# jyakaranda/A-LeGO-LOAM

Measured on AMD Instinct MI355X. Metric: scans/sec (16x1800 LiDAR) full IP->LO->LM loop, higher is better.
Workload: dtype f32/f64

## Files before the change

a-lego-loam_amd/csrc/alego_api.hip:

```cpp
#include <hip/hip_runtime.h>

#include <cmath>
#include <cstdio>
#include <cstdlib>
#include <algorithm>
#include <cstring>
#include <mutex>
#include <set>
#include <string>
#include <vector>

#include "../../include/alego_mi355x.h"
#include "dev_common.h"
#include "dev_mem.h"
#include "front_end.h"
#include "lm_ctx.h"
#include "lm_host.h"
#include "merge_math.h"
#include "thin_math.h"
#include "loop_ctx.h"
#include "pgraph.h"
#include "prof.h"
#include "reloc.h"
#include "stream_plan.h"
// ... 160 lines not shown
    h->gsize = h->plan.gsize;
    const int G = h->plan.groups;
    for (int g = 0; g < G; ++g) {
      hipStream_t s = nullptr;
      if (hipStreamCreate(&s) != hipSuccess) { for (hipStream_t t : h->streams) hipStreamDestroy(t); delete h; return ALEGO_ERR_HIP; }
      h->streams.push_back(s);
    }
    h->stream = h->streams[0];
    h->lm_async = h->plan.async != 0;
    if (h->lm_async) {
      for (int g = 0; g < G; ++g) {
        hipStream_t s = nullptr;
        hipEvent_t e[4] = {nullptr, nullptr, nullptr, nullptr};
        bool ok = hipStreamCreate(&s) == hipSuccess;
        for (int k = 0; k < 4 && ok; ++k) ok = hipEventCreateWithFlags(&e[k], hipEventDisableTiming) == hipSuccess;
        if (!ok) { h->lm_async = false; break; }
        h->back.push_back(s);
        h->ev_stage.push_back(e[0]); h->ev_stage.push_back(e[1]); h->ev_back.push_back(e[2]); h->ev_back.push_back(e[3]);
      }
      h->grp_scans.assign(G, 0);
    }
  }
  DevCtx& d = h->d;
  std::memset(&d, 0, sizeof(d));
  d.P = *params;
  d.n_slots = n_slots; d.ring_len = ring_len; d.slot0 = 0; d.n_launch = n_slots;
  d.fs_cur = d.fs_last = -1;
  d.NS = params->n_scan; d.H = params->horizon_scan; d.N = d.NS * d.H; d.Pcap = d.N;
  d.cap_sharp = params->n_sharp * params->n_sectors;
  d.cap_lsharp = params->n_less_sharp * params->n_sectors;
  d.cap_flat = params->n_flat * params->n_sectors;
  d.st_stride = d.cap_sharp + d.cap_lsharp + d.cap_flat + d.H;
  d.sin_ax = std::sin(params->seg_alpha_x); d.cos_ax = std::cos(params->seg_alpha_x);
  d.sin_ay = std::sin(params->seg_alpha_y); d.cos_ay = std::cos(params->seg_alpha_y);
  {
    const double lo = params->sensor_mount_ang - params->ground_angle_thres, hi = params->sensor_mount_ang + params->ground_angle_thres;
    const bool ok = lo > -89.0 && hi < 89.0 && lo < hi;
    d.tan_g_lo = ok ? std::tan(lo * M_PI / 180.0) : std::nan("");
    d.tan_g_hi = ok ? std::tan(hi * M_PI / 180.0) : std::nan("");
  }
  d.h_magic = (unsigned)((1ull << 32) / (unsigned long long)d.H) + 1u;
  d.inv_res_x = 1.0 / params->ang_res_x; d.inv_res_y = 1.0 / params->ang_res_y;
  d.tan_theta = (params->seg_theta > 0.0 && params->seg_theta < 1.5) ? std::tan(params->seg_theta) : std::nan("");
  d.opt_ip_screen = env_int("ALEGO_IP_SCREEN", 1) != 0;
  d.ip_scr = ip_screen_consts(d.sin_ax, d.cos_ax, d.sin_ay, d.cos_ay, d.tan_theta, d.tan_g_lo, d.tan_g_hi, d.opt_ip_screen);
  d.opt_ip_fused = env_int("ALEGO_IP_FUSED", 1) != 0;
  d.opt_ip_half = env_int("ALEGO_IP_HALF", 1) != 0;
  d.opt_cc_fused = env_int("ALEGO_CC_FUSED", 1) != 0;
  d.opt_cc_tile = env_int("ALEGO_CC_TILE", 1) != 0;
  d.opt_ip_band = env_int("ALEGO_IP_BAND", 1) != 0;
  d.opt_fe_pick1 = env_int("ALEGO_FE_PICK1", 0) != 0;
  d.opt_fe_fused = env_int("ALEGO_FE_FUSED", 1) != 0;
  d.opt_fe_cand = env_int("ALEGO_FE_CAND", 0);
  d.opt_lo_box_lds = env_int("ALEGO_LO_BOX_LDS", 1 << 20);
  d.opt_lo_grid = env_int("ALEGO_LO_GRID", 1) != 0;
  d.opt_fo_spin = env_int("ALEGO_FE_SPIN", 0);
  d.opt_fo_pad8 = env_int("ALEGO_FE_PAD8", 0) != 0;
  d.opt_map_merge = env_int("ALEGO_MAP_MERGE", 1) != 0;
  d.opt_solve_full_eval = env_int("ALEGO_SOLVE_FULL_EVAL", 0) != 0;
  d.fcap[F_SHARP] = d.cap_sharp * d.NS; d.fcap[F_LSHARP] = d.cap_lsharp * d.NS; d.fcap[F_FLAT] = d.cap_flat * d.NS; d.fcap[F_LFLAT] = d.N;
  d.lo_qcap_surf = d.fcap[F_FLAT]; d.lo_qcap_corner = d.fcap[F_SHARP];
  d.lo_box_cap = (d.N + LO_CH - 1) / LO_CH + d.NS;
  const size_t B = n_slots, N = d.N, NS = d.NS;
  int rc = 0;
  rc |= dalloc(h, &d.in_pts, B * ring_len * d.Pcap, false);
  rc |= dalloc(h, &d.in_n, B * ring_len);
  rc |= dalloc(h, &d.owner, B * N); rc |= dalloc(h, &d.range_img, B * N); rc |= dalloc(h, &d.flag_img, B * N);
  rc |= dalloc(h, &d.parent, B * N); rc |= dalloc(h, &d.cc_size, B * N); rc |= dalloc(h, &d.cc_rows, B * N);
  rc |= dalloc(h, &d.label_img, B * N); rc |= dalloc(h, &d.cc_label, B * N);
  d.ipb_col = nullptr; d.ipb_off = nullptr;
  if (d.NS > 16 && d.NS <= 64) { rc |= dalloc(h, &d.ipb_col, B * ipb_col_n(d)); rc |= dalloc(h, &d.ipb_off, B * ipb_off_n(d)); }
  d.ipf_own = nullptr;
  if (d.NS <= 16 && d.N <= 65535 && (d.H & 1) == 0) rc |= dalloc(h, &d.ipf_own, B * (N / 2), false);
  rc |= dalloc(h, &d.seg_pts, B * N); rc |= dalloc(h, &d.seg_ground, B * N); rc |= dalloc(h, &d.seg_col, B * N);
  rc |= dalloc(h, &d.seg_range, B * N); rc |= dalloc(h, &d.outlier, B * N);
  rc |= dalloc(h, &d.cd, B * N); rc |= dalloc(h, &d.picked0, B * N); rc |= dalloc(h, &d.fe_flag, B * N); rc |= dalloc(h, &d.plabel, B * N);
  rc |= fe_store_alloc(d, B, [&](auto** p, size_t n, bool zero) { return dalloc(h, p, n, zero); });
  rc |= dalloc(h, &d.scan_stamp, B);
  rc |= dalloc(h, &d.seg_dsk, h->P.deskew_mode ? B * N : 1);
  {
    const double rx = params->ang_res_x, ry = params->ang_res_y;
    std::vector<double> rt(2 * (NS + 6)), ct;
    for (int k = 0; k < (int)NS + 6; ++k) {
      const double phi = (((double)(k - 3) - 0.5) * ry - params->ang_bottom) * M_PI / 180.0;
      rt[2 * k] = std::cos(phi); rt[2 * k + 1] = std::sin(phi);
    }
    d.ip_cmin = (int)std::floor(180.0 / rx) - 2;
    d.ip_ncb = (int)std::floor(540.0 / rx) + 3 - d.ip_cmin;
    ct.resize(2 * (size_t)d.ip_ncb);
    for (int k = 0; k < d.ip_ncb; ++k) {
      const double A = (double)(d.ip_cmin + k) * rx * M_PI / 180.0;
      ct[2 * k] = std::cos(A); ct[2 * k + 1] = std::sin(A);
    }
    double2 *rtd = nullptr, *ctd = nullptr;
    rc |= dalloc(h, &rtd, NS + 6); rc |= dalloc(h, &ctd, (size_t)d.ip_ncb);
    if (!rc && (hipMemcpy(rtd, rt.data(), rt.size() * sizeof(double), hipMemcpyHostToDevice) != hipSuccess ||
                hipMemcpy(ctd, ct.data(), ct.size() * sizeof(double), hipMemcpyHostToDevice) != hipSuccess)) { h->err = "upload of the projection tables failed"; rc = ALEGO_ERR_HIP; }
    d.ip_rowtab = rtd; d.ip_coltab = ctd;
    {
      std::vector<double> cf(d.H);
      for (int c = 0; c < d.H; ++c) cf[c] = c / 10000.0;
      double* cfd = nullptr;
      rc |= dalloc(h, &cfd, (size_t)d.H);
      if (!rc && hipMemcpy(cfd, cf.data(), cf.size() * sizeof(double), hipMemcpyHostToDevice) != hipSuccess) { h->err = "upload of the column table failed"; rc = ALEGO_ERR_HIP; }
      d.ip_colfrac = cfd;
    }
// ... 641 lines not shown
  DevPool T;
  double *dg, *dp, *dr, *dj;
  HIP_TRY(h, T.get(&dg, (size_t)n * 13, false)); HIP_TRY(h, T.get(&dp, 6, false)); HIP_TRY(h, T.get(&dr, (size_t)n, false)); HIP_TRY(h, T.get(&dj, (size_t)n * 6, false));
  HIP_TRY(h, hipMemcpy(dg, geom13, (size_t)n * 13 * 8, hipMemcpyHostToDevice));
  HIP_TRY(h, hipMemcpy(dp, params6, 48, hipMemcpyHostToDevice));
  launch_dbg_eval_blocks(type, n, dg, dp, dr, dj, h->stream);
  HIP_TRY(h, hipStreamSynchronize(h->stream));
  HIP_TRY(h, hipMemcpy(res, dr, (size_t)n * 8, hipMemcpyDeviceToHost));
  HIP_TRY(h, hipMemcpy(jac6, dj, (size_t)n * 48, hipMemcpyDeviceToHost));
  return 0;
}

int alego_debug_transform_to_start(alego_handle* h, const double* params6, const alego_point* pts, int n, alego_point* out) {
  if (!h || n < 0 || !params6 || (n > 0 && (!pts || !out))) return ALEGO_ERR_ARG;
  if (n == 0) return 0;
  hipSetDevice(h->device);
  DevPool T;
  double* dp;
  float4 *di, *dout;
  HIP_TRY(h, T.get(&dp, 6, false)); HIP_TRY(h, T.get(&di, (size_t)n, false)); HIP_TRY(h, T.get(&dout, (size_t)n, false));
  HIP_TRY(h, hipMemcpy(dp, params6, 48, hipMemcpyHostToDevice));
  HIP_TRY(h, hipMemcpy(di, pts, (size_t)n * 16, hipMemcpyHostToDevice));
  launch_dbg_transform_to_start(dp, di, n, dout, h->stream);
  HIP_TRY(h, hipStreamSynchronize(h->stream));
  HIP_TRY(h, hipMemcpy(out, dout, (size_t)n * 16, hipMemcpyDeviceToHost));
  return 0;
}

int alego_debug_check_guards(char* report, int cap) {
  std::string r;
  const int bad = guard_check(&r);
  if (report && cap > 0) { std::strncpy(report, r.c_str(), (size_t)cap - 1); report[cap - 1] = 0; }
  return bad;
}

int alego_debug_set_option(alego_handle* h, const char* name, int value) {
  if (!h || !name) return ALEGO_ERR_ARG;
  const std::string s(name);
  DevCtx& d = h->d;
  if (s == "ALEGO_CC_FUSED") d.opt_cc_fused = value != 0;
  else if (s == "ALEGO_IP_FUSED") d.opt_ip_fused = value != 0;
  else if (s == "ALEGO_IP_HALF") d.opt_ip_half = value != 0;
  else if (s == "ALEGO_IP_SCREEN") { d.opt_ip_screen = value != 0; d.ip_scr = ip_screen_consts(d.sin_ax, d.cos_ax, d.sin_ay, d.cos_ay, d.tan_theta, d.tan_g_lo, d.tan_g_hi, d.opt_ip_screen); }
  else if (s == "ALEGO_CC_TILE") d.opt_cc_tile = value != 0;
  else if (s == "ALEGO_IP_BAND") {
    HIP_TRY(h, hipDeviceSynchronize());
    HIP_TRY(h, hipMemset(d.cc_size, 0, (size_t)d.n_slots * d.N * sizeof(int)));
    HIP_TRY(h, hipMemset(d.cc_rows, 0, (size_t)d.n_slots * d.N * sizeof(unsigned long long)));
    d.opt_ip_band = value != 0;
  }
  else if (s == "ALEGO_FE_PICK1") d.opt_fe_pick1 = value != 0;
  else if (s == "ALEGO_FE_FUSED") d.opt_fe_fused = value != 0;
  else if (s == "ALEGO_FE_CAND") d.opt_fe_cand = value;
  else if (s == "ALEGO_LO_BOX_LDS") d.opt_lo_box_lds = value;
  else if (s == "ALEGO_LO_GRID") d.opt_lo_grid = value != 0;
  else if (s == "ALEGO_FE_SPIN") d.opt_fo_spin = value;
  else if (s == "ALEGO_SOLVE_FULL_EVAL") d.opt_solve_full_eval = value != 0;
  else if (s == "ALEGO_FE_PAD8") d.opt_fo_pad8 = value != 0;
  else if (s == "ALEGO_FE_ERR_CLEAR") {
    if (value < -1 || value >= d.n_slots) return ALEGO_ERR_ARG;
    HIP_TRY(h, hipDeviceSynchronize());
    if (value >= 0) HIP_TRY(h, hipMemset(scal_of(d, value) + SC_FE_ERR, 0, 4));
    else HIP_TRY(h, hipMemset2D(scal_of(d, 0) + SC_FE_ERR, scal_n() * sizeof(int), 0, 4, d.n_slots));
  }
  else if (s == "ALEGO_MAP_MERGE") { if (int r = lm_host_set_map_merge(h->lm, value != 0, &h->err)) return r; d.opt_map_merge = value != 0; }
  else if (s == "ALEGO_IP_FAST") d.ip_fast = h->ip_fast_capable & value;
  else if (s == "ALEGO_POKE_GUARD") { HIP_TRY(h, hipMemset(scal_of(d, d.n_slots) + value, 0xFF, 4)); }
  else if (s == "ALEGO_GV_SMALL_MAX") { HIP_TRY(h, sync_all(h)); return lm_host_set_gv_small_max(h->lm, value); }
  else if (s == "ALEGO_PG_BUDGET") graph_ctx_set_budget(&h->pg, value);
  else if (s == "ALEGO_LC_BUDGET") loop_ctx_set_budget(&h->lc, value);
  else if (s == "ALEGO_RL_BUDGET") reloc_ctx_set(&h->rl, 0, value);
  else if (s == "ALEGO_RL_BRUTE") reloc_ctx_set(&h->rl, 1, value);
  else if (s == "ALEGO_SHARD_SLICE") return lm_host_debug_slice(h->lm, value & 0xff, value >> 8, &h->err);
  else { h->err = "unknown option " + s; return ALEGO_ERR_ARG; }
  return 0;
}

int alego_loop_detect(const alego_params* P, const float* keyposes6, const double* stamps, int32_t n, const double cur_xyz[3]) {
  if (!P || n <= 0 || !keyposes6 || !stamps || !cur_xyz) return -1;
  const float cx = (float)cur_xyz[0], cy = (float)cur_xyz[1], cz = (float)cur_xyz[2];
  const float r2 = (float)(P->lc_search_radius * P->lc_search_radius);
  std::vector<std::pair<float, int>> cand;
  for (int i = 0; i < n; ++i) {
    float r = 0.f, df;
    df = keyposes6[i * 6 + 0] - cx; r += df * df; df = keyposes6[i * 6 + 1] - cy; r += df * df; df = keyposes6[i * 6 + 2] - cz; r += df * df;
    if (r < r2) cand.emplace_back(r, i);
  }
  std::sort(cand.begin(), cand.end());
  for (const auto& c : cand)
    if (stamps[n - 1] - stamps[c.second] > P->lc_min_time_gap) return c.second;
  return -1;
}
int alego_loop_closure_icp(alego_handle* h, const alego_kf_in* latest, const alego_kf_in* history, int32_t n_history, alego_icp_result* out,
                           alego_point* target_out, int32_t target_cap) {
  if (!h || !latest || !out || n_history < 0 || (n_history > 0 && !history)) return ALEGO_ERR_ARG;
  hipSetDevice(h->device);
  g_prof = &h->prof;
  return icp_run(h->P, latest, history, n_history, out, target_out, target_out ? target_cap : 0, h->stream, &h->err);
}

int alego_loop_search(alego_handle* h, const int32_t* slots, int32_t n, alego_loop_result* out) {
  if (!h || n < 0 || (n > 0 && (!slots || !out))) return ALEGO_ERR_ARG;
  if (!h->map_on) { h->err = "alego_loop_search: the key-frame archive is off (alego_map_enable)"; return ALEGO_ERR_ARG; }
  for (int i = 0; i < n; ++i) if (slots[i] < 0 || slots[i] >= h->d.n_slots) { h->err = "alego_loop_search: slot out of range"; return ALEGO_ERR_ARG; }
  hipSetDevice(h->device);
  g_prof = &h->prof;
// ... 537 lines not shown
  hipSetDevice(h->device);
  return lm_host_map_stamps(h->lm, slot, first, n, const_cast<double*>(stamps), 1, &h->err);
}
int alego_map_keyposes(alego_handle* h, int slot, alego_point* out, int32_t cap) {
  if (int r = check_slot(h, slot)) return r;
  hipSetDevice(h->device);
  return lm_host_map_keyposes(h->lm, slot, out, cap, &h->err);
}
int alego_lm_get_local_map(alego_handle* h, int slot, alego_point* corner, int32_t corner_cap, alego_point* surf, int32_t surf_cap, int32_t n_out[2]) {
  if (int r = check_slot(h, slot)) return r;
  if (!n_out || corner_cap < 0 || surf_cap < 0) return ALEGO_ERR_ARG;
  hipSetDevice(h->device);
  return lm_host_get_local_map(h->lm, slot, corner, corner_cap, surf, surf_cap, n_out, &h->err);
}
int alego_voxel_grid(alego_handle* h, const alego_point* pts, int32_t n, float leaf, alego_point* out, int32_t cap) {
  if (!h || n < 0 || cap < 0 || (n > 0 && !pts) || !(leaf > 0.f)) return ALEGO_ERR_ARG;
  hipSetDevice(h->device);
  g_prof = &h->prof;
  return lm_host_voxel_grid(h->lm, h->stream, pts, n, leaf, out, cap, &h->err);
}

int alego_debug_get(alego_handle* h, int slot, const char* name, void* out, int cap_bytes, int* count, int* dtype) {
  if (int r = check_slot(h, slot)) return r;
  hipSetDevice(h->device);
  const DevCtx& d = h->d;
  int sc[SC_COUNT];
  HIP_TRY(h, hipMemcpyAsync(sc, scal_of(d, slot), sizeof(sc), hipMemcpyDeviceToHost, stream_of(h, slot)));
  HIP_TRY(h, hipStreamSynchronize(stream_of(h, slot)));
  const std::string s(name);
  if (s.rfind("la_", 0) == 0) {
    const void* rsrc = nullptr;
    size_t bytes = 0;
    if (loop_app_debug_get(h->rl, slot, name, &rsrc, &bytes)) { h->err = std::string("debug_get: ") + name + " needs alego_loop_appearance_enable"; return ALEGO_ERR_ARG; }
    if ((size_t)cap_bytes < bytes) { h->err = "debug_get: buffer too small"; return ALEGO_ERR_CAPACITY; }
    if (bytes) HIP_TRY(h, hipMemcpy(out, rsrc, bytes, hipMemcpyDeviceToHost));
    *count = (int)bytes; *dtype = 3;
    return 0;
  }
  if (s.rfind("rl_", 0) == 0) {
    if (s == "rl_stats") {
      if (cap_bytes < 8) { h->err = "debug_get: buffer too small"; return ALEGO_ERR_CAPACITY; }
      reloc_debug_stats(h->rl, (int*)out);
      *count = 2; *dtype = 2;
      return 0;
    }
    const void* rsrc = nullptr;
    size_t bytes = 0;
    if (reloc_debug_get(h->rl, slot, name, &rsrc, &bytes)) { h->err = std::string("debug_get: ") + name + " needs alego_reloc_enable"; return ALEGO_ERR_ARG; }
    if ((size_t)cap_bytes < bytes) { h->err = "debug_get: buffer too small"; return ALEGO_ERR_CAPACITY; }
    if (bytes) HIP_TRY(h, hipMemcpy(out, rsrc, bytes, hipMemcpyDeviceToHost));
    *count = (int)bytes; *dtype = 3;
    return 0;
  }
  const size_t base = (size_t)slot * d.N, M = sc[SC_M];
  const size_t fb = fbuf(slot, sc[SC_CUR]);
  int fc[F_KINDS];
  HIP_TRY(h, hipMemcpy(fc, feat_cnt_of(d, fb), sizeof(fc), hipMemcpyDeviceToHost));
  static const char* const cloud[F_KINDS] = {"sharp", "less_sharp", "flat", "less_flat"};
  struct Row { std::string name; const void* row; size_t n; int dtype; };
  std::vector<Row> tab = {
    {"range_img", d.range_img + base, (size_t)d.N, 0}, {"label_img", d.label_img + base, (size_t)d.N, 2}, {"flag_img", d.flag_img + base, (size_t)d.N, 3},
    {"owner", d.owner + base, (size_t)d.N, 2}, {"parent", d.parent + base, (size_t)d.N, 2},
    {"seg_cloud", d.seg_pts + base, M * 4, 0}, {"outlier", d.outlier + base, (size_t)sc[SC_NOUT] * 4, 0},
    {"imu_ptr", imu_ptr_of(d, slot), IMP_N, 2}, {"imu_ring", imu_ring_of(d, slot), imu_ring_n(), 1},
    {"seg_ground", d.seg_ground + base, M, 3}, {"seg_col", d.seg_col + base, M, 2}, {"seg_range", d.seg_range + base, M, 0},
    {"ring_start", ring_start_of(d, slot, 0), (size_t)d.NS, 2}, {"ring_end", ring_end_of(d, slot, 0), (size_t)d.NS, 2},
    {"orientation", ori_of(d, slot), ORI_N, 0}, {"scal", scal_of(d, slot), SC_COUNT, 2},
    {"curv_d", d.cd + base, M, 0}, {"picked_occl", d.picked0 + base, M, 3}, {"point_label", d.plabel + base, M, 2},
    {"lo_surf_corr", lo_corr_of(d, slot, 0), (size_t)fc[F_FLAT] * LC_W, 2}, {"lo_corner_corr", lo_corr_of(d, slot, 1), (size_t)fc[F_SHARP] * LC_W, 2},
    {"lo_state", lo_state_of(d, slot), LO_STATE_N, 1}, {"poses", poses_of(d, slot), PO_W, 1}};
  if (d.P.deskew_mode) tab.push_back({"undistorted", d.seg_dsk + base, (size_t)sc[SC_M_DSK] * 4, 0});
  for (int k = 0; k < F_KINDS; ++k) {
    tab.push_back({cloud[k], feat_of(d, k, fb), (size_t)fc[k] * 4, 0});
    if (k < F_LFLAT) tab.push_back({std::string(cloud[k]) + "_idx", feat_idx_of(d, k, fb), (size_t)fc[k], 2});
  }
  const Row* hit = nullptr;
  for (const Row& r : tab) if (r.name == s) hit = &r;
  if (!hit) return lm_host_debug_get(h->lm, slot, name, out, cap_bytes, count, dtype, &h->err);
  const void* src = hit->row;
  const size_t n = hit->n, esz = hit->dtype == 1 ? 8 : hit->dtype == 3 ? 1 : 4;
  const int dt = hit->dtype;
  if ((size_t)cap_bytes < n * esz) { h->err = "debug_get: buffer too small"; return ALEGO_ERR_CAPACITY; }
  if (n) HIP_TRY(h, hipMemcpy(out, src, n * esz, hipMemcpyDeviceToHost));
  *count = (int)n; *dtype = dt;
  return 0;
}

}
```

a-lego-loam_amd/csrc/dev_common.h:

```cpp
#ifndef ALEGO_DEV_COMMON_H_
#define ALEGO_DEV_COMMON_H_

#include <hip/hip_runtime.h>
#include <stdint.h>

#include "../../include/alego_params.h"
#include "wave.h"
#include "ip_pred.h"

#define IPB_NM 9
#define IP_OWNER_TAG 0x40000000

struct DevCtx {
  alego_params P;
  int n_slots, ring_len;
  int slot0, n_launch;
  int N, H, NS;
  int Pcap;
  int cap_sharp, cap_lsharp, cap_flat;
  double sin_ax, cos_ax, sin_ay, cos_ay;
  double inv_res_x, inv_res_y;
  const double2* ip_rowtab;
  const double2* ip_coltab;
  const double* ip_colfrac;
  int ip_cmin, ip_ncb, ip_fast;
  unsigned h_magic;
  double tan_g_lo, tan_g_hi;
  double tan_theta;
  IpScreenConsts ip_scr;
  int opt_ip_fused;
  int opt_ip_half;
  int opt_cc_fused;
  int opt_cc_tile;
  int opt_fe_pick1;
  int opt_fe_fused;
  int opt_fe_cand;
  int opt_lo_box_lds;
  int opt_map_merge;
  int opt_ip_screen;
  int opt_solve_full_eval;
  float4* in_pts;
  int* in_n;
  const float4* bag_pts;
  const int* bag_n;
  const int2* bag_src;
  int n_bags, bag_len, replay_bag;
  int fs_cur, fs_last;
  int* owner;
  float* range_img;
  uint8_t* flag_img;
  int* parent;
  int* cc_size;
  unsigned long long* cc_rows;
  unsigned long long* ipb_col;
  int* ipb_off;
  int opt_ip_band;
  unsigned* ipf_own;
  int* label_img;
  int* cc_label;
  int* row_cnt;
  int* scal;
  float4* seg_pts;
  uint8_t* seg_ground;
  int* seg_col;
  float* seg_range;
  int* ring_start;
  int* ring_end;
  float* ori;
  float4* outlier;
  float* cd;
  uint8_t* picked0;
  uint8_t* fe_flag;
  int* plabel;
  int* st_idx;
  int* st_cnt;
  float4* st_lfds;
  int st_stride;
  float4* feat[4];
  int* feat_idx[3];
  int fcap[4];
  int* feat_cnt;
  int* ring_off;
  int* ring_boff;
  unsigned* fe_sync;
  int* lo_corr;
  int lo_qcap_surf, lo_qcap_corner;
  float4* lo_box;
  float4* lo_cpts[2];
  unsigned short* lo_cell;
// ... 135 lines not shown
```

a-lego-loam_amd/csrc/front_end.h:

```cpp
#ifndef ALEGO_FRONT_END_H_
#define ALEGO_FRONT_END_H_
#include "dev_common.h"

void launch_ip(const DevCtx& d, int ring_pos, bool want_labels, hipStream_t st);
void launch_atan2f_probe(const float* y, const float* x, float* out, int n, int mode, hipStream_t st);
int ip_configure(const DevCtx& d);
bool ipf_eligible(const DevCtx& d), ipw_eligible(const DevCtx& d), ipb_eligible(const DevCtx& d);
void launch_ip_fused(const DevCtx& d, int ring_pos, bool keep_images, hipStream_t st);
int ipf_configure(const DevCtx& d);
void launch_ipb(const DevCtx& d, int ring_pos, bool keep_images, hipStream_t st);
void launch_fe(const DevCtx& d, hipStream_t st);
void launch_fe_curv_debug(const DevCtx& d, hipStream_t st);
int launch_stdsort_probe(const uint32_t* keys, int n, int depth_limit, int* pos_out, hipStream_t st);
bool fe_fused_eligible(const DevCtx& d);
void launch_fe_fused(const DevCtx& d, hipStream_t st);
void launch_lo(const DevCtx& d, hipStream_t st);
void launch_lo_grid(const DevCtx& d, hipStream_t st);
void launch_lo_imu_push(const DevCtx& d, int slot, const double* smp_dev, int n, hipStream_t st);
void launch_lo_deskew(const DevCtx& d, hipStream_t st);
void launch_traj_log(const DevCtx& d, hipStream_t st, const double* staged_odom = nullptr, int par = 0);
void launch_dbg_eval_blocks(int type, int n, const double* geom13, const double* params6, double* res, double* jac6, hipStream_t st);
void launch_dbg_transform_to_start(const double* params6, const float4* pts, int n, float4* out, hipStream_t st);
int lo_configure();
#endif
```

a-lego-loam_amd/csrc/kernels_fe2.hip:

```cpp
#include <algorithm>
#include <cstdlib>
#include "dev_common.h"
#include "front_end.h"
#include "prof.h"
#include "vgrid.h"

#define FE_MAXH 4096

#ifndef FF_G
#define FF_G 4
#endif
#define FF_LPR (64 / FF_G)
#define FF_HALO 8
#define FF_Q0 64
#ifndef FC_NW
#define FC_NW 4
#endif

struct FfLayout {
  int scap, mch, wave_bytes;
};
__host__ __device__ inline FfLayout ff_layout(int sector_cap) {
  FfLayout L;
  L.scap = (FF_Q0 + sector_cap + FF_HALO + 63) & ~63;
  L.mch = L.scap / 64 + 1;
  L.wave_bytes = (8 * 4 * L.mch + 4 * L.scap + 2 * L.scap + 7) & ~7;
  return L;
}

DEV_INLINE unsigned long long ext128(unsigned long long lo, unsigned long long hi, int pos) { return (lo >> pos) | (pos ? hi << (64 - pos) : 0ull); }

DEV_INLINE void ff_sector(const alego_params& P, int S, int E, int j, int& sp, int& ep) {
  const int NSEC = P.n_sectors;
  if (NSEC == 6) {
    if (P.sector_formula == 0) { sp = (S * (6 - j) + E * j) / 6; ep = (S * (5 - j) + E * (j + 1)) / 6 - 1; }
    else { const int diff = E - S; sp = S + j * diff / 6; ep = S + (j + 1) * diff / 6 - 1; }
    return;
  }
  if (P.sector_formula == 0) { sp = (S * (NSEC - j) + E * j) / NSEC; ep = (S * (NSEC - 1 - j) + E * (j + 1)) / NSEC - 1; }
  else { const int diff = E - S; sp = S + j * diff / NSEC; ep = S + (j + 1) * diff / NSEC - 1; }
}

DEV_INLINE uint2* ff_list(const DevCtx& d, int slot, int ring, int j, int sector_cap) {
  return st_cand_of(d, slot, ring) + (size_t)j * sector_cap;
}
DEV_INLINE int* ff_counts(const DevCtx& d, int slot, int ring) {
  return st_idx_of(d, slot, ring, F_LFLAT);
}

DEV_INLINE void ff_wide(const DevCtx& d, size_t base, int M, int sp, int ep, unsigned char* wl, const FfLayout& L, uint2* list, int sector_cap, int& ns_out, int& nf_out, bool dbg) {
  const int lane = threadIdx.x & 63;
  const alego_params& P = d.P;
  unsigned long long* mA = reinterpret_cast<unsigned long long*>(wl);
  unsigned long long* mB = mA + L.mch, *mC = mB + L.mch, *mJ = mC + L.mch;
  float* sr = reinterpret_cast<float*>(wl + 8 * 4 * L.mch);
  uint16_t* scl = reinterpret_cast<uint16_t*>(wl + 8 * 4 * L.mch + 4 * L.scap);
  const float* rng = d.seg_range + base;
  const int* colv = d.seg_col + base;
  const uint8_t* gndv = d.seg_ground + base;
  const int len = ep - sp + 1;
  const int q0 = FF_Q0 - FF_HALO, q1 = FF_Q0 + len + FF_HALO;
#pragma unroll 2
  for (int q = q0 + lane; q < q1; q += 64) {
    const int k = sp + q - FF_Q0;
    const bool in = k >= 0 && k < M;
    const unsigned ku = in ? (unsigned)k : 0u;
    const float r = rng[ku];
    const int c = colv[ku];
    const uint8_t g = gndv[ku];
    sr[q] = in ? r : 0.f;
    scl[q] = in ? (uint16_t)((c & 0x7fff) | (g ? 0x8000 : 0)) : (uint16_t)0;
  }
  __syncthreads();
  const int nch = (q1 + 63) >> 6;
  for (int ch = 0; ch < nch; ++ch) {
    const int q = ch * 64 + lane, k = sp + q - FF_Q0;
    const bool inr = q > q0 && q < q1 - 1;
    const int qa = min(max(q, q0 + 1), q1 - 2);
    const float r0 = sr[qa], r1 = sr[qa + 1], rm = sr[qa - 1];
    const int c0 = scl[qa] & 0x7fff, c1 = scl[qa + 1] & 0x7fff;
    int cdiff = c0 - c1;
    cdiff = cdiff < 0 ? -cdiff : cdiff;
    bool c1b, c2b;
    double diff1, diff2;
    if (P.occl_f32) {
      c1b = (double)(r0 - r1) > P.occl_depth; c2b = (double)(r1 - r0) > P.occl_depth;
      diff1 = (double)fabsf(rm - r0); diff2 = (double)fabsf(r1 - r0);
    } else {
      const double d1 = (double)r0, d2 = (double)r1;
      c1b = d1 - d2 > P.occl_depth; c2b = d2 - d1 > P.occl_depth;
      diff1 = fabs((double)rm - d1); diff2 = fabs(d2 - d1);
    }
    const bool okp = inr && k >= 5 && k < M - 5;
    const bool near = cdiff < P.occl_col_diff;
    const bool A = okp && near && c1b;
    const bool B = okp && near && !c1b && c2b;
    const bool C = okp && !A && diff1 > P.parallel_ratio * (double)r0 && diff2 > P.parallel_ratio * (double)r0;
    const bool J = inr && k + 1 < M && cdiff > P.suppress_col_diff;
    const unsigned long long a = __ballot(A), b = __ballot(B), c = __ballot(C), j = __ballot(J);
    if (lane == 0) { mA[ch] = a; mB[ch] = b; mC[ch] = c; mJ[ch] = j; }
  }
  __syncthreads();
  int ns = 0, nf = 0;
  const int SR = P.suppress_radius;
  for (int it = 0; it * 64 < len; ++it) {
    const int ch = it + 1, q = ch * 64 + lane, loc = it * 64 + lane, k = sp + loc;
    const bool own = loc < len;
    const bool gnd = (scl[q] & 0x8000) != 0;
    const float cdv = sr[q - 5] + sr[q - 4] + sr[q - 3] + sr[q - 2] + sr[q - 1] - sr[q] * 10 + sr[q + 1] + sr[q + 2] + sr[q + 3] + sr[q + 4] + sr[q + 5];
    const unsigned long long a0 = mA[ch], a1 = ch + 1 < nch ? mA[ch + 1] : 0ull;
    const unsigned long long bp = mB[ch - 1], b0 = mB[ch];
    const unsigned long long j0 = mJ[ch], j1 = ch + 1 < nch ? mJ[ch + 1] : 0ull, jp = mJ[ch - 1];
    const bool anyA = (ext128(a0, a1, lane) & 0x3full) != 0;
    const bool anyB = (ext128((bp >> 59) | (b0 << 5), b0 >> 59, lane) & 0x1full) != 0;
    const bool pk = ((mC[ch] >> lane) & 1ull) || anyA || anyB;
    const unsigned f5 = (unsigned)(ext128(j0, j1, lane) & 0x1full);
    const unsigned w5 = (unsigned)(ext128((jp >> 59) | (j0 << 5), j0 >> 59, lane) & 0x1full);
    const int rf = min(SR, __ffs((int)(f5 | 0x20u)) - 1), rb = min(SR, __clz((int)(w5 << 27)));
    const double ad = (double)fabsf(cdv), curv = ad * ad;
    const bool free_ = own && !pk;
    const bool cs = free_ && !gnd && curv > P.edge_thres;
    const bool cf = free_ && gnd && curv < P.surf_thres;
    const uint32_t kb = (uint32_t)d_f2i(fabsf(cdv));
    const uint32_t pay = ((uint32_t)loc << 6) | ((uint32_t)rf << 3) | (uint32_t)rb;
    const unsigned long long ms = __ballot(cs), mf = __ballot(cf), below = (1ull << lane) - 1ull;
    if (cs) list[(unsigned)(ns + (int)__popcll(ms & below))] = make_uint2(kb + 1u, pay);
    if (cf) list[(unsigned)(sector_cap - 1 - (nf + (int)__popcll(mf & below)))] = make_uint2(~kb, ~pay);
    ns += (int)__popcll(ms); nf += (int)__popcll(mf);
    if (dbg && own) { d.cd[base + k] = cdv; d.picked0[base + k] = pk ? 1 : 0; }
  }
  ns_out = ns; nf_out = nf;
}

__global__ void __launch_bounds__(64 * FC_NW) fe_cand(DevCtx d, int sector_cap) {
  const int slot = blockIdx.y + d.slot0, lane = threadIdx.x & 63, wave = __builtin_amdgcn_readfirstlane((int)(threadIdx.x >> 6));
  const int NS = d.NS, NSEC = d.P.n_sectors;
  const int item = blockIdx.x * FC_NW + wave, ring = item / NSEC, j = item - ring * NSEC;
  const size_t base = (size_t)slot * d.N;
  const int M = scal_of(d, slot)[SC_M];
  extern __shared__ __attribute__((aligned(16))) unsigned char ff_smem[];
  const FfLayout L = ff_layout(sector_cap);
  int sp = 0, ep = -1;
  if (ring < NS) ff_sector(d.P, *ring_start_of(d, slot, ring), *ring_end_of(d, slot, ring), j, sp, ep);
  int ns = 0, nf = 0;
  if (sp < ep) ff_wide(d, base, M, sp, ep, ff_smem + wave * L.wave_bytes, L, ff_list(d, slot, ring, j, sector_cap), sector_cap, ns, nf, d.n_launch == 1);
  else { __syncthreads(); __syncthreads(); }
  if (ring < NS && lane == 0) { int* cc = ff_counts(d, slot, ring); cc[2 * j] = ns; cc[2 * j + 1] = nf; }
}

struct FfPick {
  bool act0;
  int sp;
  int carry;
  int carry_in;
  int n_sharp, n_ls, n_flat;
  int* st_sharp; int* st_lsharp; int* st_flat;
};

template <bool FLAT>
DEV_INLINE void ff_label(const alego_params& P, int picked, int nmax, int& lab, bool& spread, bool& more) {
  if (FLAT) { lab = -1; more = picked < P.n_flat; spread = more; }
  else { lab = picked <= P.n_sharp ? 2 : (picked <= P.n_less_sharp ? 1 : 0); spread = lab != 0; more = lab != 0 && picked < nmax; }
}
template <bool FLAT>
DEV_INLINE void ff_commit(FfPick& R, bool rem, int lab, int c, int lo, int hi, uint32_t* mark, int mw, int gl) {
  if (!FLAT) {
    const int w = (lo >> 5) + (gl & 1), wl = max(lo, 32 * w), wh = min(hi, 32 * w + 31);
    const uint32_t bits = (rem && gl < 2 && wh >= wl) ? (((2u << (wh - 32 * w)) - 1u) & ~((1u << (wl - 32 * w)) - 1u)) : 0u;
    atomicOr(&mark[min(w, mw - 1)], bits);
  }
  if (rem) R.carry = max(R.carry, R.sp + hi);
  if (rem && gl == 0) {
    if (FLAT) R.st_flat[R.n_flat] = R.sp + c;
    else { if (lab == 2) R.st_sharp[R.n_sharp] = R.sp + c; R.st_lsharp[R.n_ls] = R.sp + c; }
  }
  if (FLAT) R.n_flat += rem ? 1 : 0;
  else { R.n_sharp += (rem && lab == 2) ? 1 : 0; R.n_ls += rem ? 1 : 0; }
}
DEV_INLINE bool ff_marked(const uint32_t* mark, int mw, uint32_t loc) { return (mark[min((int)(loc >> 5), mw - 1)] >> (loc & 31u)) & 1u; }

template <int K, bool FLAT>
DEV_INLINE void ff_pick_regs(const alego_params& P, FfPick& R, int ncand, const uint2* lp, int dir, uint32_t* mark, int mw, int gl) {
  uint32_t key[K], pay[K];
#pragma unroll
  for (int t = 0; t < K; ++t) {
    const int idx = gl + FF_LPR * t;
    const bool ok = R.act0 && idx < ncand;
    const uint2 e = lp[(ok ? idx : 0) * dir];
    const uint32_t pv = FLAT ? ~e.y : e.y, loc = pv >> 6;
    const bool gone = R.sp + (int)loc <= R.carry_in || (FLAT && ff_marked(mark, mw, loc));
    key[t] = (ok && !gone) ? e.x : 0u; pay[t] = e.y;
  }
  const int nmax = FLAT ? 0x7fffffff : max(P.n_sharp, P.n_less_sharp);
  int picked = 0;
  bool act = R.act0 && (FLAT || nmax > 0);
  while (true) {
    uint32_t bk = 0u, bp = 0u;
#pragma unroll
    for (int t = 0; t < K; ++t) {
      const bool take = FLAT ? key[t] > bk : key[t] >= bk;
// ... 576 lines not shown
      c[3 * FO_MAXBOX] = fo_ord(hi3[0]); c[4 * FO_MAXBOX] = fo_ord(hi3[1]); c[5 * FO_MAXBOX] = fo_ord(hi3[2]);
    }
  } else {
    for (int b = tid; b < 6 * FO_MAXBOX; b += FO_BLOCK) s_bx[b] = b < 3 * FO_MAXBOX ? 0xFFFFFFFFu : 0u;
    __syncthreads();
    FO_TICK(13);
#pragma nounroll
    for (int c = 0; c * FO_BLOCK < nrv; ++c) {
      const int j = c * FO_BLOCK + tid;
      const uint32_t a0 = j < nrv ? s_tmp[j] : 0x1000u;
      const bool head = !(a0 & 0x1000u);
      const unsigned long long m = __ballot(head);
      const int rank0 = __builtin_amdgcn_readlane(vex, __builtin_amdgcn_readfirstlane(c * NW + wv));
      if (head) {
        const int rank = rank0 + (int)__popcll(m & lt);
        int i = (int)(a0 & 0xFFFu);
        float4 q = point(i);
        float sx = 0.f, sy = 0.f, sz = 0.f, si = 0.f;
        int cnt = 0;
#pragma nounroll
        for (;;) {
          const int ni = s_nxt[i];
          sx += q.x; sy += q.y; sz += q.z; si += q.w; ++cnt;
          if (ni == FO_END) break;
          q = point(ni); i = ni;
        }
        const float fn = (float)cnt;
        const float4 ctr = make_float4(sx / fn, sy / fn, sz / fn, si / fn);
        out[rank] = ctr;
        box_add(rank, ctr);
      }
    }
  }
  __syncthreads();
  FO_TICK(7);
  {
    float4* bx = lo_box_of(d, lo_row(fb, box_set_of(F_LFLAT))) + (size_t)2 * boff3;
    for (int b = tid; b < nbox; b += FO_BLOCK) {
      const uint32_t* c = s_bx + b;
      bx[2 * b] = make_float4(fo_unord(c[0]), fo_unord(c[FO_MAXBOX]), fo_unord(c[2 * FO_MAXBOX]), __int_as_float(off3 + b * LO_CH));
      bx[2 * b + 1] = make_float4(fo_unord(c[3 * FO_MAXBOX]), fo_unord(c[4 * FO_MAXBOX]), fo_unord(c[5 * FO_MAXBOX]), __int_as_float(min(LO_CH, nout - b * LO_CH)));
    }
    if (tid == 0) {
      int* ro = ring_off_of(d, fb, RO_LFLAT);
      int* rb = ring_boff_of(d, fb, RO_LFLAT);
      ro[ring] = off3; rb[ring] = boff3;
      if (ring == NS - 1) { ro[NS] = off3 + nout; rb[NS] = boff3 + nbox; feat_cnt_of(d, fb)[F_LFLAT] = off3 + nout; }
      st_cnt_of(d, slot, ring)[ST_LFDS] = nout;
    }
  }
  FO_TICK(8);
}

bool fe_fused_eligible(const DevCtx& d) {
  const int nsec = d.P.n_sectors;
  if (!(d.opt_fe_fused && !d.opt_fe_pick1 && d.P.sort_mode != 2 && d.NS <= 64 && d.H <= FE_MAXH && nsec >= 1)) return false;
  const long long sector_cap = (d.H + nsec - 1) / nsec + 2;
  return nsec <= FO_BLOCK && (long long)nsec * sector_cap <= 2LL * d.H && 2LL * nsec <= d.H;
}

void launch_fe_fused(const DevCtx& d, hipStream_t st) {
  static const bool cfg = hipFuncSetAttribute(reinterpret_cast<const void*>(fe_ring_out), hipFuncAttributeMaxDynamicSharedMemorySize, (int)fo_lds_bytes(FE_MAXH)) == hipSuccess;
  (void)cfg;
  const int sector_cap = (d.H + d.P.n_sectors - 1) / (d.P.n_sectors > 0 ? d.P.n_sectors : 1) + 2;
  if (d.n_launch == 1) launch_fe_curv_debug(d, st);
  const FfLayout L = ff_layout(sector_cap);
  ALEGO_LAUNCH(fe_cand, dim3((d.NS * d.P.n_sectors + FC_NW - 1) / FC_NW, d.n_launch), dim3(64 * FC_NW), (size_t)FC_NW * L.wave_bytes, st, d, sector_cap);
  const dim3 gp((d.NS + FF_G - 1) / FF_G, d.n_launch);
  if (sector_cap > 400) { ALEGO_LAUNCH(fe_pickc<true>, gp, dim3(64), 0, st, d, sector_cap); }
  else { ALEGO_LAUNCH(fe_pickc<false>, gp, dim3(64), 0, st, d, sector_cap); }
  ALEGO_LAUNCH(fe_ring_out, dim3(d.opt_fo_pad8 ? (d.n_launch + 7) / 8 * 8 : d.n_launch, d.NS + 1), dim3(FO_BLOCK), fo_lds_bytes(d.H), st, d);
}
```

Baseline: 485,800.

## Stream feature candidates per ring through a rolling LDS window, one wave per ring

The candidate kernel changes from one wavefront per sector to, by default, one wavefront per whole ring that walks all of that ring's sectors. Points are staged through a fixed 256-column circular LDS window with halo, using register prefetch and wave-level barriers instead of block barriers, so dynamic LDS sized by sector length is no longer needed. Neighbour-sector halos are read once instead of once per sector, and the per-sector list and count outputs are written as the wave crosses sector boundaries. The trade is fewer, longer waves, which lowers parallelism (NS waves per slot instead of NS*n_sectors) in exchange for less redundant loading and a smaller static LDS footprint.

```diff
diff --git a/a-lego-loam_amd/csrc/alego_api.hip b/a-lego-loam_amd/csrc/alego_api.hip
--- a/a-lego-loam_amd/csrc/alego_api.hip
+++ b/a-lego-loam_amd/csrc/alego_api.hip
@@ -236,6 +236,7 @@
   d.opt_fe_pick1 = env_int("ALEGO_FE_PICK1", 0) != 0;
   d.opt_fe_fused = env_int("ALEGO_FE_FUSED", 1) != 0;
   d.opt_fe_cand = env_int("ALEGO_FE_CAND", 0);
+  d.opt_fe_span = env_int("ALEGO_FE_SPAN", 0);
   d.opt_lo_box_lds = env_int("ALEGO_LO_BOX_LDS", 1 << 20);
   d.opt_lo_grid = env_int("ALEGO_LO_GRID", 1) != 0;
   d.opt_fo_spin = env_int("ALEGO_FE_SPIN", 0);
@@ -983,6 +984,7 @@
   else if (s == "ALEGO_FE_PICK1") d.opt_fe_pick1 = value != 0;
   else if (s == "ALEGO_FE_FUSED") d.opt_fe_fused = value != 0;
   else if (s == "ALEGO_FE_CAND") d.opt_fe_cand = value;
+  else if (s == "ALEGO_FE_SPAN") d.opt_fe_span = value;
   else if (s == "ALEGO_LO_BOX_LDS") d.opt_lo_box_lds = value;
   else if (s == "ALEGO_LO_GRID") d.opt_lo_grid = value != 0;
   else if (s == "ALEGO_FE_SPIN") d.opt_fo_spin = value;
@@ -1626,6 +1628,23 @@
     *count = (int)bytes; *dtype = 3;
     return 0;
   }
+  if (s == "fe_cand_span") {
+    if (cap_bytes < 8) { h->err = "debug_get: buffer too small"; return ALEGO_ERR_CAPACITY; }
+    ((int*)out)[0] = fe_cand_span(d); ((int*)out)[1] = fe_sector_cap(d);
+    *count = 2; *dtype = 2;
+    return 0;
+  }
+  if (s == "fe_cand_counts" || s == "fe_cand_lists") {
+    if (!fe_fused_eligible(d)) { h->err = "debug_get: " + s + " needs the fused feature extraction"; return ALEGO_ERR_ARG; }
+    const bool lists = s == "fe_cand_lists";
+    const size_t row = lists ? (size_t)d.P.n_sectors * fe_sector_cap(d) * sizeof(uint2) : (size_t)d.P.n_sectors * 2 * sizeof(int);
+    const void* src = lists ? (const void*)st_cand_of(d, slot, 0) : (const void*)st_idx_of(d, slot, 0, F_LFLAT);
+    const size_t pitch = lists ? (size_t)((const char*)st_cand_of(d, slot, 1) - (const char*)st_cand_of(d, slot, 0)) : (size_t)((const char*)st_idx_of(d, slot, 1, F_LFLAT) - (const char*)st_idx_of(d, slot, 0, F_LFLAT));
+    if ((size_t)cap_bytes < row * d.NS) { h->err = "debug_get: buffer too small"; return ALEGO_ERR_CAPACITY; }
+    HIP_TRY(h, hipMemcpy2D(out, row, src, pitch, row, d.NS, hipMemcpyDeviceToHost));
+    *count = (int)(row * d.NS / 4); *dtype = 2;
+    return 0;
+  }
   const size_t base = (size_t)slot * d.N, M = sc[SC_M];
   const size_t fb = fbuf(slot, sc[SC_CUR]);
   int fc[F_KINDS];
diff --git a/a-lego-loam_amd/csrc/dev_common.h b/a-lego-loam_amd/csrc/dev_common.h
--- a/a-lego-loam_amd/csrc/dev_common.h
+++ b/a-lego-loam_amd/csrc/dev_common.h
@@ -35,6 +35,7 @@
   int opt_fe_pick1;
   int opt_fe_fused;
   int opt_fe_cand;
+  int opt_fe_span;
   int opt_lo_box_lds;
   int opt_map_merge;
   int opt_ip_screen;
diff --git a/a-lego-loam_amd/csrc/front_end.h b/a-lego-loam_amd/csrc/front_end.h
--- a/a-lego-loam_amd/csrc/front_end.h
+++ b/a-lego-loam_amd/csrc/front_end.h
@@ -13,6 +13,8 @@
 void launch_fe_curv_debug(const DevCtx& d, hipStream_t st);
 int launch_stdsort_probe(const uint32_t* keys, int n, int depth_limit, int* pos_out, hipStream_t st);
 bool fe_fused_eligible(const DevCtx& d);
+int fe_cand_span(const DevCtx& d);
+int fe_sector_cap(const DevCtx& d);
 void launch_fe_fused(const DevCtx& d, hipStream_t st);
 void launch_lo(const DevCtx& d, hipStream_t st);
 void launch_lo_grid(const DevCtx& d, hipStream_t st);
diff --git a/a-lego-loam_amd/csrc/kernels_fe2.hip b/a-lego-loam_amd/csrc/kernels_fe2.hip
--- a/a-lego-loam_amd/csrc/kernels_fe2.hip
+++ b/a-lego-loam_amd/csrc/kernels_fe2.hip
@@ -12,33 +12,35 @@
 #endif
 #define FF_LPR (64 / FF_G)
 #define FF_HALO 8
-#define FF_Q0 64
+#ifndef FC_SPAN
+#define FC_SPAN 0
+#endif
 #ifndef FC_NW
 #define FC_NW 4
 #endif
+#define FF_WIN 256
 
 struct FfLayout {
-  int scap, mch, wave_bytes;
+  int cols, wave_bytes;
 };
-__host__ __device__ inline FfLayout ff_layout(int sector_cap) {
-  FfLayout L;
-  L.scap = (FF_Q0 + sector_cap + FF_HALO + 63) & ~63;
-  L.mch = L.scap / 64 + 1;
-  L.wave_bytes = (8 * 4 * L.mch + 4 * L.scap + 2 * L.scap + 7) & ~7;
-  return L;
-}
+__host__ __device__ constexpr FfLayout ff_layout() {
+  return FfLayout{4 * (FF_WIN + 2 * FF_HALO), (4 + 2) * (FF_WIN + 2 * FF_HALO)};
+}
+static_assert(ff_layout().wave_bytes % 8 == 0, "a wavefront's LDS slice keeps the alignment of the first");
 
 DEV_INLINE unsigned long long ext128(unsigned long long lo, unsigned long long hi, int pos) { return (lo >> pos) | (pos ? hi << (64 - pos) : 0ull); }
 
-DEV_INLINE void ff_sector(const alego_params& P, int S, int E, int j, int& sp, int& ep) {
+DEV_INLINE int ff_sector_start(const alego_params& P, int S, int E, int j) {
   const int NSEC = P.n_sectors;
   if (NSEC == 6) {
-    if (P.sector_formula == 0) { sp = (S * (6 - j) + E * j) / 6; ep = (S * (5 - j) + E * (j + 1)) / 6 - 1; }
-    else { const int diff = E - S; sp = S + j * diff / 6; ep = S + (j + 1) * diff / 6 - 1; }
-    return;
-  }
-  if (P.sector_formula == 0) { sp = (S * (NSEC - j) + E * j) / NSEC; ep = (S * (NSEC - 1 - j) + E * (j + 1)) / NSEC - 1; }
-  else { const int diff = E - S; sp = S + j * diff / NSEC; ep = S + (j + 1) * diff / NSEC - 1; }
+    if (P.sector_formula == 0) return (S * (6 - j) + E * j) / 6;
+    return S + j * (E - S) / 6;
+  }
+  if (P.sector_formula == 0) return (S * (NSEC - j) + E * j) / NSEC;
+  return S + j * (E - S) / NSEC;
+}
+DEV_INLINE void ff_sector(const alego_params& P, int S, int E, int j, int& sp, int& ep) {
+  sp = ff_sector_start(P, S, E, j); ep = ff_sector_start(P, S, E, j + 1) - 1;
 }
 
 DEV_INLINE uint2* ff_list(const DevCtx& d, int slot, int ring, int j, int sector_cap) {
@@ -48,37 +50,54 @@
   return st_idx_of(d, slot, ring, F_LFLAT);
 }
 
-DEV_INLINE void ff_wide(const DevCtx& d, size_t base, int M, int sp, int ep, unsigned char* wl, const FfLayout& L, uint2* list, int sector_cap, int& ns_out, int& nf_out, bool dbg) {
+DEV_INLINE unsigned long long ff_ballot(bool p) { return __builtin_amdgcn_ballot_w64(p); }
+DEV_INLINE void ff_wave_sync() {
+  __builtin_amdgcn_fence(__ATOMIC_RELEASE, "wavefront");
+  __builtin_amdgcn_wave_barrier();
+  __builtin_amdgcn_fence(__ATOMIC_ACQUIRE, "wavefront");
+}
+
+DEV_INLINE void ff_span(const DevCtx& d, size_t base, int M, int S, int E, int j0, int j1, unsigned char* wl, uint2* list, int* cc, int sector_cap, bool dbg) {
   const int lane = threadIdx.x & 63;
   const alego_params& P = d.P;
-  unsigned long long* mA = reinterpret_cast<unsigned long long*>(wl);
-  unsigned long long* mB = mA + L.mch, *mC = mB + L.mch, *mJ = mC + L.mch;
-  float* sr = reinterpret_cast<float*>(wl + 8 * 4 * L.mch);
-  uint16_t* scl = reinterpret_cast<uint16_t*>(wl + 8 * 4 * L.mch + 4 * L.scap);
+  constexpr FfLayout L = ff_layout();
+  float* sr = reinterpret_cast<float*>(wl) + FF_HALO;
+  uint16_t* scl = reinterpret_cast<uint16_t*>(wl + L.cols) + FF_HALO;
   const float* rng = d.seg_range + base;
   const int* colv = d.seg_col + base;
   const uint8_t* gndv = d.seg_ground + base;
-  const int len = ep - sp + 1;
-  const int q0 = FF_Q0 - FF_HALO, q1 = FF_Q0 + len + FF_HALO;
-#pragma unroll 2
-  for (int q = q0 + lane; q < q1; q += 64) {
-    const int k = sp + q - FF_Q0;
+  const int lo = ff_sector_start(P, S, E, j0), hi = ff_sector_start(P, S, E, j1) - 1;
+  const int len = hi - lo + 1;
+  if (len < 2) {
+    for (int j = j0 + lane; j < j1; j += 64) { cc[2 * j] = 0; cc[2 * j + 1] = 0; }
+    return;
+  }
+  const int q1 = len + 2 * FF_HALO;
+  const int nc = (FF_HALO + len + 63) >> 6;
+  const unsigned long long below = (1ull << lane) - 1ull;
+  const int SR = P.suppress_radius;
+
+  auto fetch = [&](int t, float& r, int& c, uint8_t& g) {
+    const int k = lo + t * 64 + lane - FF_HALO;
+    const unsigned ku = (k >= 0 && k < M) ? (unsigned)k : 0u;
+    r = rng[ku]; c = colv[ku]; g = gndv[ku];
+  };
+  auto stage = [&](int t, float r, int c, uint8_t g) {
+    const int k = lo + t * 64 + lane - FF_HALO;
     const bool in = k >= 0 && k < M;
-    const unsigned ku = in ? (unsigned)k : 0u;
-    const float r = rng[ku];
-    const int c = colv[ku];
-    const uint8_t g = gndv[ku];
-    sr[q] = in ? r : 0.f;
-    scl[q] = in ? (uint16_t)((c & 0x7fff) | (g ? 0x8000 : 0)) : (uint16_t)0;
-  }
-  __syncthreads();
-  const int nch = (q1 + 63) >> 6;
-  for (int ch = 0; ch < nch; ++ch) {
-    const int q = ch * 64 + lane, k = sp + q - FF_Q0;
-    const bool inr = q > q0 && q < q1 - 1;
-    const int qa = min(max(q, q0 + 1), q1 - 2);
-    const float r0 = sr[qa], r1 = sr[qa + 1], rm = sr[qa - 1];
-    const int c0 = scl[qa] & 0x7fff, c1 = scl[qa + 1] & 0x7fff;
+    const float rv = in ? r : 0.f;
+    const uint16_t cv = in ? (uint16_t)((c & 0x7fff) | (g ? 0x8000 : 0)) : (uint16_t)0;
+    const int w = t & 3, p = w * 64 + lane;
+    sr[p] = rv; scl[p] = cv;
+    if (w == 0 && lane < FF_HALO) { sr[p + FF_WIN] = rv; scl[p + FF_WIN] = cv; }
+    if (w == 3 && lane >= 64 - FF_HALO) { sr[p - FF_WIN] = rv; scl[p - FF_WIN] = cv; }
+  };
+  auto marks = [&](int m, unsigned long long& a, unsigned long long& b, unsigned long long& c, unsigned long long& j) {
+    const int q = m * 64 + lane, k = lo + q - FF_HALO;
+    const bool inr = q > 0 && q < q1 - 1;
+    const int pa = (m & 3) * 64 + lane;
+    const float r0 = sr[pa], r1 = sr[pa + 1], rm = sr[pa - 1];
+    const int c0 = scl[pa] & 0x7fff, c1 = scl[pa + 1] & 0x7fff;
     int cdiff = c0 - c1;
     cdiff = cdiff < 0 ? -cdiff : cdiff;
     bool c1b, c2b;
@@ -97,55 +116,81 @@
     const bool B = okp && near && !c1b && c2b;
     const bool C = okp && !A && diff1 > P.parallel_ratio * (double)r0 && diff2 > P.parallel_ratio * (double)r0;
     const bool J = inr && k + 1 < M && cdiff > P.suppress_col_diff;
-    const unsigned long long a = __ballot(A), b = __ballot(B), c = __ballot(C), j = __ballot(J);
-    if (lane == 0) { mA[ch] = a; mB[ch] = b; mC[ch] = c; mJ[ch] = j; }
-  }
-  __syncthreads();
-  int ns = 0, nf = 0;
-  const int SR = P.suppress_radius;
-  for (int it = 0; it * 64 < len; ++it) {
-    const int ch = it + 1, q = ch * 64 + lane, loc = it * 64 + lane, k = sp + loc;
-    const bool own = loc < len;
-    const bool gnd = (scl[q] & 0x8000) != 0;
-    const float cdv = sr[q - 5] + sr[q - 4] + sr[q - 3] + sr[q - 2] + sr[q - 1] - sr[q] * 10 + sr[q + 1] + sr[q + 2] + sr[q + 3] + sr[q + 4] + sr[q + 5];
-    const unsigned long long a0 = mA[ch], a1 = ch + 1 < nch ? mA[ch + 1] : 0ull;
-    const unsigned long long bp = mB[ch - 1], b0 = mB[ch];
-    const unsigned long long j0 = mJ[ch], j1 = ch + 1 < nch ? mJ[ch + 1] : 0ull, jp = mJ[ch - 1];
+    a = ff_ballot(A); b = ff_ballot(B); c = ff_ballot(C); j = ff_ballot(J);
+  };
+
+  float fr = 0.f, fr1 = 0.f, fr2 = 0.f;
+  int fc = 0, fc1 = 0, fc2 = 0;
+  uint8_t fg = 0, fg1 = 0, fg2 = 0;
+  fetch(0, fr, fc, fg);
+  if (64 < q1) fetch(1, fr1, fc1, fg1);
+  if (128 < q1) fetch(2, fr2, fc2, fg2);
+  stage(0, fr, fc, fg);
+  if (64 < q1) stage(1, fr1, fc1, fg1);
+  if (128 < q1) stage(2, fr2, fc2, fg2);
+  if (192 < q1) fetch(3, fr, fc, fg);
+  ff_wave_sync();
+  unsigned long long bp = 0ull, jp = 0ull, a0, b0, c0m, j0m, a1 = 0ull, b1 = 0ull, c1m = 0ull, j1m = 0ull;
+  marks(0, a0, b0, c0m, j0m);
+  int jc = j0, spc = lo, nxt = ff_sector_start(P, S, E, j0 + 1), ns = 0, nf = 0;
+  for (int c = 0; c < nc; ++c) {
+    ff_wave_sync();
+    if ((c + 1) * 64 < q1) marks(c + 1, a1, b1, c1m, j1m);
+    else { a1 = 0ull; b1 = 0ull; c1m = 0ull; j1m = 0ull; }
+    const int q = c * 64 + lane, k = lo + q - FF_HALO, p = (c & 3) * 64 + lane;
+    const bool gnd = (scl[p] & 0x8000) != 0;
+    const float cdv = sr[p - 5] + sr[p - 4] + sr[p - 3] + sr[p - 2] + sr[p - 1] - sr[p] * 10 + sr[p + 1] + sr[p + 2] + sr[p + 3] + sr[p + 4] + sr[p + 5];
     const bool anyA = (ext128(a0, a1, lane) & 0x3full) != 0;
     const bool anyB = (ext128((bp >> 59) | (b0 << 5), b0 >> 59, lane) & 0x1full) != 0;
-    const bool pk = ((mC[ch] >> lane) & 1ull) || anyA || anyB;
-    const unsigned f5 = (unsigned)(ext128(j0, j1, lane) & 0x1full);
-    const unsigned w5 = (unsigned)(ext128((jp >> 59) | (j0 << 5), j0 >> 59, lane) & 0x1full);
+    const bool pk = ((c0m >> lane) & 1ull) || anyA || anyB;
+    const unsigned f5 = (unsigned)(ext128(j0m, j1m, lane) & 0x1full);
+    const unsigned w5 = (unsigned)(ext128((jp >> 59) | (j0m << 5), j0m >> 59, lane) & 0x1full);
     const int rf = min(SR, __ffs((int)(f5 | 0x20u)) - 1), rb = min(SR, __clz((int)(w5 << 27)));
     const double ad = (double)fabsf(cdv), curv = ad * ad;
-    const bool free_ = own && !pk;
-    const bool cs = free_ && !gnd && curv > P.edge_thres;
-    const bool cf = free_ && gnd && curv < P.surf_thres;
+    const bool cs0 = !pk && !gnd && curv > P.edge_thres;
+    const bool cf0 = !pk && gnd && curv < P.surf_thres;
     const uint32_t kb = (uint32_t)d_f2i(fabsf(cdv));
-    const uint32_t pay = ((uint32_t)loc << 6) | ((uint32_t)rf << 3) | (uint32_t)rb;
-    const unsigned long long ms = __ballot(cs), mf = __ballot(cf), below = (1ull << lane) - 1ull;
-    if (cs) list[(unsigned)(ns + (int)__popcll(ms & below))] = make_uint2(kb + 1u, pay);
-    if (cf) list[(unsigned)(sector_cap - 1 - (nf + (int)__popcll(mf & below)))] = make_uint2(~kb, ~pay);
-    ns += (int)__popcll(ms); nf += (int)__popcll(mf);
+    const uint32_t reach = ((uint32_t)rf << 3) | (uint32_t)rb;
+    const int klast = lo + c * 64 + 63 - FF_HALO;
+    ff_wave_sync();
+    if ((c + 3) * 64 < q1) stage(c + 3, fr, fc, fg);
+    if ((c + 4) * 64 < q1) fetch(c + 4, fr, fc, fg);
+    bool own = false;
+    while (true) {
+      const bool in = k >= spc && k < nxt && nxt - spc >= 2;
+      const bool cs = cs0 && in, cf = cf0 && in;
+      const uint32_t pay = ((uint32_t)(k - spc) << 6) | reach;
+      const unsigned long long ms = ff_ballot(cs), mf = ff_ballot(cf);
+      if (cs) list[(unsigned)(ns + (int)__popcll(ms & below))] = make_uint2(kb + 1u, pay);
+      if (cf) list[(unsigned)(sector_cap - 1 - (nf + (int)__popcll(mf & below)))] = make_uint2(~kb, ~pay);
+      ns += (int)__popcll(ms); nf += (int)__popcll(mf);
+      own = own || in;
+      if (nxt > klast || jc + 1 >= j1) break;
+      if (lane == 0) { cc[2 * jc] = ns; cc[2 * jc + 1] = nf; }
+      ++jc; spc = nxt; nxt = ff_sector_start(P, S, E, jc + 1); ns = 0; nf = 0; list += sector_cap;
+    }
     if (dbg && own) { d.cd[base + k] = cdv; d.picked0[base + k] = pk ? 1 : 0; }
-  }
-  ns_out = ns; nf_out = nf;
-}
-
+    bp = b0; jp = j0m; a0 = a1; b0 = b1; c0m = c1m; j0m = j1m;
+  }
+  if (lane == 0) {
+    cc[2 * jc] = ns; cc[2 * jc + 1] = nf;
+    for (int j = jc + 1; j < j1; ++j) { cc[2 * j] = 0; cc[2 * j + 1] = 0; }
+  }
+}
+
+template <int SPAN>
 __global__ void __launch_bounds__(64 * FC_NW) fe_cand(DevCtx d, int sector_cap) {
-  const int slot = blockIdx.y + d.slot0, lane = threadIdx.x & 63, wave = __builtin_amdgcn_readfirstlane((int)(threadIdx.x >> 6));
+  const int slot = blockIdx.y + d.slot0, wave = __builtin_amdgcn_readfirstlane((int)(threadIdx.x >> 6));
   const int NS = d.NS, NSEC = d.P.n_sectors;
-  const int item = blockIdx.x * FC_NW + wave, ring = item / NSEC, j = item - ring * NSEC;
+  const int nspan = SPAN > 0 ? (NSEC + SPAN - 1) / SPAN : 1;
+  const int item = blockIdx.x * FC_NW + wave, ring = item / nspan, s = item - ring * nspan;
+  if (ring >= NS) return;
+  const int j0 = SPAN > 0 ? s * SPAN : 0, j1 = SPAN > 0 ? min(j0 + SPAN, NSEC) : NSEC;
   const size_t base = (size_t)slot * d.N;
   const int M = scal_of(d, slot)[SC_M];
-  extern __shared__ __attribute__((aligned(16))) unsigned char ff_smem[];
-  const FfLayout L = ff_layout(sector_cap);
-  int sp = 0, ep = -1;
-  if (ring < NS) ff_sector(d.P, *ring_start_of(d, slot, ring), *ring_end_of(d, slot, ring), j, sp, ep);
-  int ns = 0, nf = 0;
-  if (sp < ep) ff_wide(d, base, M, sp, ep, ff_smem + wave * L.wave_bytes, L, ff_list(d, slot, ring, j, sector_cap), sector_cap, ns, nf, d.n_launch == 1);
-  else { __syncthreads(); __syncthreads(); }
-  if (ring < NS && lane == 0) { int* cc = ff_counts(d, slot, ring); cc[2 * j] = ns; cc[2 * j + 1] = nf; }
+  __shared__ __attribute__((aligned(16))) unsigned char ff_smem[FC_NW * ff_layout().wave_bytes];
+  ff_span(d, base, M, *ring_start_of(d, slot, ring), *ring_end_of(d, slot, ring), j0, j1, ff_smem + wave * ff_layout().wave_bytes,
+          ff_list(d, slot, ring, j0, sector_cap), ff_counts(d, slot, ring), sector_cap, d.n_launch == 1);
 }
 
 struct FfPick {
@@ -828,20 +873,25 @@
   FO_TICK(8);
 }
 
+int fe_sector_cap(const DevCtx& d) { return (d.H + d.P.n_sectors - 1) / (d.P.n_sectors > 0 ? d.P.n_sectors : 1) + 2; }
+int fe_cand_span(const DevCtx& d) { return d.opt_fe_span == 1 ? 1 : FC_SPAN; }
+
 bool fe_fused_eligible(const DevCtx& d) {
   const int nsec = d.P.n_sectors;
   if (!(d.opt_fe_fused && !d.opt_fe_pick1 && d.P.sort_mode != 2 && d.NS <= 64 && d.H <= FE_MAXH && nsec >= 1)) return false;
-  const long long sector_cap = (d.H + nsec - 1) / nsec + 2;
+  const long long sector_cap = fe_sector_cap(d);
   return nsec <= FO_BLOCK && (long long)nsec * sector_cap <= 2LL * d.H && 2LL * nsec <= d.H;
 }
 
 void launch_fe_fused(const DevCtx& d, hipStream_t st) {
   static const bool cfg = hipFuncSetAttribute(reinterpret_cast<const void*>(fe_ring_out), hipFuncAttributeMaxDynamicSharedMemorySize, (int)fo_lds_bytes(FE_MAXH)) == hipSuccess;
   (void)cfg;
-  const int sector_cap = (d.H + d.P.n_sectors - 1) / (d.P.n_sectors > 0 ? d.P.n_sectors : 1) + 2;
+  const int sector_cap = fe_sector_cap(d);
   if (d.n_launch == 1) launch_fe_curv_debug(d, st);
-  const FfLayout L = ff_layout(sector_cap);
-  ALEGO_LAUNCH(fe_cand, dim3((d.NS * d.P.n_sectors + FC_NW - 1) / FC_NW, d.n_launch), dim3(64 * FC_NW), (size_t)FC_NW * L.wave_bytes, st, d, sector_cap);
+  const int nsec = d.P.n_sectors, nspan = (d.opt_fe_span == 1 || FC_SPAN == 1) ? nsec : (FC_SPAN > 0 ? (nsec + FC_SPAN - 1) / FC_SPAN : 1);
+  const dim3 gc((d.NS * nspan + FC_NW - 1) / FC_NW, d.n_launch);
+  if (d.opt_fe_span == 1) { ALEGO_LAUNCH(fe_cand<1>, gc, dim3(64 * FC_NW), 0, st, d, sector_cap); }
+  else { ALEGO_LAUNCH(fe_cand<FC_SPAN>, gc, dim3(64 * FC_NW), 0, st, d, sector_cap); }
   const dim3 gp((d.NS + FF_G - 1) / FF_G, d.n_launch);
   if (sector_cap > 400) { ALEGO_LAUNCH(fe_pickc<true>, gp, dim3(64), 0, st, d, sector_cap); }
   else { ALEGO_LAUNCH(fe_pickc<false>, gp, dim3(64), 0, st, d, sector_cap); }
```

Measured after the change: 491,700 (median of 6 runs). 1.01x the previous value.
